# yuecideng/Misc3D

Hardware: AMD Instinct MI355X
Metric: RANSAC hypotheses/sec, 1M-pt cloud (inlier-score GB/s: roofline.algorithmic_reuse) (higher is better)
Workload: dtype f64 decisions (fp32 screen + fp64 recount)

## Files before the change

include/misc3d_amd_bench.h:

```cpp
#ifndef MISC3D_AMD_BENCH_H
#define MISC3D_AMD_BENCH_H

#include "misc3d_amd.h"

#ifdef __cplusplus
extern "C" {
#endif

int m3d_bench_time_score(m3d_cloud *cloud, int kind, double threshold, const uint32_t *samples,
                         size_t n_hypotheses, int reps, int mode, double *ms_avg,
                         uint64_t *listed_pairs);


int m3d_bench_fp64_issue_rate(int device, double ms_target, double *tera_lane_ops_per_s, double *ms_measured);

int m3d_bench_cloud_setup_ms(const m3d_cloud *cloud, double out[5]);

int m3d_bench_plane_upper_bounds(m3d_cloud *cloud, double threshold, const uint32_t *samples, size_t n_hypotheses,
                                 uint32_t *ub_out);
int m3d_bench_plane_ref_upper_bounds(m3d_cloud *cloud, double threshold, const uint32_t *samples, size_t n_hypotheses,
                                     size_t ref_index, uint32_t *ub_out);
int m3d_bench_upper_bounds(m3d_cloud *cloud, int kind, double threshold, const uint32_t *samples, size_t n_hypotheses,
                           uint32_t *ub_out);
int m3d_bench_last_segment_ms(double out[6]);

int m3d_bench_reg_checkers(const double *ps, const double *pd, const double *T, double edge_threshold,
                           double distance_threshold);

int m3d_bench_kabsch_sums(const double *src, const double *dst, size_t n, int device, double out[18]);

int m3d_bench_icp_sums(const double *src, size_t n_src, const double *dst, size_t n_dst, double max_correspondence_distance,
                       const double *T, int device, double out[29], int64_t *corr);

int m3d_bench_fps_force_path(int path);

int m3d_bench_knn_force_path(int path);

int m3d_bench_knn_tile_merge(const double *data, size_t n, int dim, const double *queries, size_t m, int kk, int pages,
                             int splits, uint32_t rows_per_split, int device, uint32_t *idx_out, uint64_t *d2_bits_out);

int m3d_bench_voxel_force_path(int path);

int m3d_bench_proximity_cutoffs(double dist, double angle_deg, double out[5]);

int m3d_bench_radius_grid_geom(const double lo[3], const double hi[3], double edge, int K0, int *K, double *h, uint64_t dims[3]);
int m3d_bench_reg_grid_k0(int k_cfg, uint64_t n_dst);

int m3d_bench_fpfh_pair_bins(const double *pairs, size_t m, int32_t *bins, double *features);

int m3d_bench_fpfh_stages(const double *xyz, const double *normals, size_t n, int search, double radius, int max_nn, int device,
                          uint32_t *list_idx, double *list_d2, uint32_t *cnt, uint8_t *spfh_count, double *spfh_incr,
                          uint32_t *tie_points, uint64_t *n_ties, double *feature_out, m3d_fpfh_stats *stats);

unsigned m3d_bench_match_last_path(void);

int m3d_bench_ppf_force(int device_memory_path, int max_groups);

int m3d_bench_ppf_cluster_force(int splits);

int m3d_bench_scratch_fill(int pattern);
int m3d_bench_scratch_fill_stats(uint64_t out[2]);
int m3d_bench_scratch_probe(int device, size_t bytes, unsigned char first_last[128]);

#ifdef __cplusplus
}
#endif
#endif
```

misc3d_amd/csrc/m3d_bench_hooks.cpp:

```cpp
#include "m3d_driver_internal.hpp"

#pragma clang fp contract(off)

using namespace m3d;

extern "C" {

int m3d_bench_last_segment_ms(double out[6]) {
    if (!out) return fail(M3D_ERR_INVALID_ARG, "null argument");
    for (int k = 0; k < 6; ++k) out[k] = g_seg_ms[k];
    return M3D_OK;
}

int m3d_bench_radius_grid_geom(const double lo[3], const double hi[3], double edge, int K0, int* K, double* h, uint64_t dims[3]) {
    if (!lo || !hi || !K || !h || !dims || !(edge > 0.0) || K0 < 1 || K0 > 16)
        return fail(M3D_ERR_INVALID_ARG, "invalid argument");
    const RadiusGridGeom g = radius_grid_geom(lo, hi, edge, K0);
    *K = g.K;
    *h = g.h;
    for (int k = 0; k < 3; ++k) dims[k] = g.dims[k];
    return M3D_OK;
}

int m3d_bench_reg_grid_k0(int k_cfg, uint64_t n_dst) { return reg_grid_k0(k_cfg, n_dst); }

int m3d_bench_cloud_setup_ms(const m3d_cloud* c, double out[5]) {
    if (!c || !out) return fail(M3D_ERR_INVALID_ARG, "null argument");
    for (int k = 0; k < 5; ++k) out[k] = c->setup_ms[k];
    return M3D_OK;
}

int m3d_bench_fp64_issue_rate(int device, double ms_target, double* tops, double* ms_measured) {
    if (!tops) return fail(M3D_ERR_INVALID_ARG, "invalid argument");
    LaneLock lane(device);
    DeviceCtx* ctx = lane.ctx;
    if (!ctx) return M3D_ERR_DEVICE;
    HIPCHK(hipSetDevice(ctx->device));
    RESERVE(ctx->small, 256);
    const int blocks = 256 * 8;
    auto run = [&](int iters, float* ms) -> int {
        HIPCHK(hipEventRecord(ctx->ev0, ctx->stream));
        launch_fp64_issue_probe(ctx->small.as<double>(), blocks, iters, ctx->stream);
        HIPCHK(hipEventRecord(ctx->ev1, ctx->stream));
        HIPCHK(hipGetLastError());
        HIPCHK(hipStreamSynchronize(ctx->stream));
        HIPCHK(hipEventElapsedTime(ms, ctx->ev0, ctx->ev1));
        return M3D_OK;
    };
    float ms = 0;
    int rc = run(256, &ms);
    if (rc != M3D_OK) return rc;
    rc = run(2048, &ms);
    if (rc != M3D_OK) return rc;
    const double per_iter = (double)ms / 2048.0;
    const int iters = (int)std::min(4.0e6, std::max(1024.0, (ms_target > 0 ? ms_target : 2.0) / std::max(per_iter, 1e-9)));
    rc = run(iters, &ms);
    if (rc != M3D_OK) return rc;
    const double ops = (double)blocks * 256.0 * 16.0 * (double)iters;
    *tops = ops / ((double)ms * 1e-3) / 1e12;
    if (ms_measured) *ms_measured = ms;
    return M3D_OK;
}

}
```

misc3d_amd/csrc/m3d_mask_expand.hpp:

```cpp
#pragma once

#include <cstddef>
#include <cstdint>
#include <thread>
#include <vector>

#if defined(__x86_64__)
#include <immintrin.h>
#endif

namespace m3d {

constexpr uint32_t kMaskTileWords = 32;

inline uint64_t mask_tile_prefix(const uint32_t* counts, uint32_t nb, uint64_t* prefix) {
    uint64_t s = 0;
    for (uint32_t t = 0; t < nb; ++t) {
        prefix[t] = s;
        s += counts[t];
    }
    prefix[nb] = s;
    return s;
}

inline void mask_split(const uint64_t* prefix, uint32_t nb, uint32_t parts, uint32_t* bounds) {
    const uint64_t total = prefix[nb];
    bounds[0] = 0;
    uint32_t t = 0;
    for (uint32_t k = 1; k < parts; ++k) {
        const uint64_t want = total * k / parts;
        while (t < nb && prefix[t] < want) ++t;
        bounds[k] = t;
    }
    bounds[parts] = nb;
}

namespace mask_detail {

inline uint64_t word_at(const uint64_t* mask, uint64_t w, uint64_t n) {
    const uint64_t m = mask[w];
    const uint64_t first = w * 64;
    return n - first >= 64 ? m : (m & ((1ull << (n - first)) - 1ull));
}

inline bool expand_scalar(const uint64_t* mask, uint64_t n, const uint64_t* prefix, uint32_t t0, uint32_t t1, uint64_t* dst) {
    const uint64_t n_words = (n + 63) / 64;
    for (uint32_t t = t0; t < t1; ++t) {
        uint64_t pos = prefix[t];
        const uint64_t end = prefix[t + 1];
        const uint64_t w0 = (uint64_t)t * kMaskTileWords, w1 = w0 + kMaskTileWords < n_words ? w0 + kMaskTileWords : n_words;
        for (uint64_t w = w0; w < w1; ++w) {
            uint64_t m = word_at(mask, w, n);
            if (!m) continue;
            if (pos + (uint64_t)__builtin_popcountll(m) > end) return false;
            const uint64_t b = w * 64;
            do {
                dst[pos++] = b + (uint64_t)__builtin_ctzll(m);
                m &= m - 1;
            } while (m);
        }
        if (pos != end) return false;
    }
    return true;
}

#if defined(__x86_64__)
__attribute__((target("avx512f,popcnt"))) inline bool expand_avx512(const uint64_t* mask, uint64_t n, const uint64_t* prefix,
                                                                uint32_t t0, uint32_t t1, uint64_t* dst) {
    const uint64_t n_words = (n + 63) / 64;
    const __m512i lane = _mm512_set_epi64(7, 6, 5, 4, 3, 2, 1, 0);
    const __m512i eight = _mm512_set1_epi64(8);
    for (uint32_t t = t0; t < t1; ++t) {
        uint64_t pos = prefix[t];
        const uint64_t end = prefix[t + 1];
        const uint64_t w0 = (uint64_t)t * kMaskTileWords, w1 = w0 + kMaskTileWords < n_words ? w0 + kMaskTileWords : n_words;
        for (uint64_t w = w0; w < w1; ++w) {
            const uint64_t m = word_at(mask, w, n);
            if (!m) continue;
            const uint64_t pc = (uint64_t)_mm_popcnt_u64(m);
            if (pos + pc > end) return false;
            __m512i v = _mm512_add_epi64(_mm512_set1_epi64((long long)(w * 64)), lane);
            uint64_t* d = dst + pos;
            if (m == ~0ull) {
                for (int k = 0; k < 8; ++k) {
                    _mm512_storeu_si512(d + 8 * k, v);
                    v = _mm512_add_epi64(v, eight);
                }
            } else {
                for (int k = 0; k < 8; ++k) {
                    const __mmask8 s = (__mmask8)(m >> (8 * k));
                    if (s) {
                        const __m512i c = _mm512_maskz_compress_epi64(s, v);
                        const unsigned c_n = (unsigned)_mm_popcnt_u32(s);
                        _mm512_mask_storeu_epi64(d, (__mmask8)((1u << c_n) - 1u), c);
                        d += c_n;
                    }
                    v = _mm512_add_epi64(v, eight);
                }
            }
            pos += pc;
        }
        if (pos != end) return false;
    }
    return true;
}
#endif

}

inline bool mask_have_avx512() {
#if defined(__x86_64__)
    static const bool have = __builtin_cpu_supports("avx512f") && __builtin_cpu_supports("popcnt");
    return have;
#else
    return false;
#endif
}

inline bool mask_expand_range(const uint64_t* mask, uint64_t n, const uint64_t* prefix, uint32_t t0, uint32_t t1, uint64_t* dst,
                              int path = -1) {
#if defined(__x86_64__)
    if (path != 0 && mask_have_avx512()) return mask_detail::expand_avx512(mask, n, prefix, t0, t1, dst);
#endif
    return mask_detail::expand_scalar(mask, n, prefix, t0, t1, dst);
}

inline bool mask_expand_threads(const uint64_t* mask, uint64_t n, const uint32_t* counts, uint64_t* dst, uint32_t writers,
                                int path = -1) {
    const uint32_t nb = (uint32_t)((n + 64ull * kMaskTileWords - 1) / (64ull * kMaskTileWords));
    if (writers < 1) writers = 1;
    std::vector<uint64_t> prefix(nb + 1);
    mask_tile_prefix(counts, nb, prefix.data());
    std::vector<uint32_t> bounds(writers + 1);
    mask_split(prefix.data(), nb, writers, bounds.data());
    std::vector<char> ok(writers, 1);
    std::vector<std::thread> th;
    for (uint32_t k = 1; k < writers; ++k)
        th.emplace_back([&, k] { ok[k] = mask_expand_range(mask, n, prefix.data(), bounds[k], bounds[k + 1], dst, path); });
    ok[0] = mask_expand_range(mask, n, prefix.data(), bounds[0], bounds[1], dst, path);
    for (auto& t : th) t.join();
    for (char c : ok)
        if (!c) return false;
    return true;
}

}
```

misc3d_amd/csrc/m3d_refine.cpp:

```cpp
#include "m3d_driver_internal.hpp"
#include "m3d_generalfit_fp.hpp"
#include "m3d_mask_expand.hpp"

#include <condition_variable>
#include <mutex>
#include <sched.h>

#pragma clang fp contract(off)

namespace m3d {

namespace {
class MaskPool {
public:
    static MaskPool& get() {
        static MaskPool* p = new MaskPool();
        return *p;
    }
    static uint32_t writer_cap() {
        const int lm = config().list_mask;
        uint32_t cap = lm >= 2 ? (uint32_t)lm : 8u;
        cpu_set_t set;
        CPU_ZERO(&set);
        if (sched_getaffinity(0, sizeof(set), &set) == 0) cap = std::min<uint32_t>(cap, (uint32_t)std::max(CPU_COUNT(&set), 1));
        return std::max<uint32_t>(cap, 1u);
    }
    void arm() {
        const uint32_t helpers = writer_cap() - 1;
        spin_us_.store(std::max(config().wait_spin_us, 0), std::memory_order_relaxed);
        if (helpers == 0) return;
        std::lock_guard<std::mutex> lk(mu_);
        try {
            while (threads_ < helpers) {
                std::thread(&MaskPool::helper, this, threads_).detach();
                ++threads_;
            }
        } catch (...) {
        }
        want_ = std::min(helpers, threads_);
        arm_seq_.fetch_add(1, std::memory_order_release);
        if (parked_) cv_.notify_all();
    }
    bool expand(const uint64_t* mask, uint64_t n, const uint32_t* counts, uint64_t* dst) {
        const uint32_t nb = (uint32_t)((n + 64ull * kMaskTileWords - 1) / (64ull * kMaskTileWords));
        if (nb == 0) return true;
        bool expected = false;
        if (!busy_.compare_exchange_strong(expected, true, std::memory_order_acquire)) {
            std::vector<uint64_t> prefix(nb + 1);
            mask_tile_prefix(counts, nb, prefix.data());
            return mask_expand_range(mask, n, prefix.data(), 0, nb, dst);
        }
        prefix_.resize(nb + 1);
        mask_tile_prefix(counts, nb, prefix_.data());
        const uint32_t ranges = std::min<uint32_t>(nb, 4u * writer_cap());
        bounds_.resize(ranges + 1);
        mask_split(prefix_.data(), nb, ranges, bounds_.data());
        mask_ = mask;
        n_ = n;
        dst_ = dst;
        failed_.store(false, std::memory_order_relaxed);
        done_.store(0, std::memory_order_relaxed);
        job_.store((uint64_t)ranges << 32, std::memory_order_release);
        work();
        while (done_.load(std::memory_order_acquire) != ranges) {
#if defined(__x86_64__) || defined(__i386__)
            __builtin_ia32_pause();
#endif
        }
        const bool ok = !failed_.load(std::memory_order_relaxed);
        busy_.store(false, std::memory_order_release);
        return ok;
    }

private:
    bool work() {
        bool any = false;
        for (;;) {
            const uint64_t v = job_.load(std::memory_order_relaxed);
            if ((v & 0xFFFFFFFFull) >= (v >> 32)) return any;
            const uint64_t c = job_.fetch_add(1, std::memory_order_acq_rel);
            const uint32_t k = (uint32_t)c, ranges = (uint32_t)(c >> 32);
            if (k >= ranges) return any;
            if (!mask_expand_range(mask_, n_, prefix_.data(), bounds_[k], bounds_[k + 1], dst_))
                failed_.store(true, std::memory_order_relaxed);
            done_.fetch_add(1, std::memory_order_release);
            any = true;
        }
    }
    void helper(uint32_t id) {
        uint64_t seen = 0;
        for (;;) {
            {
                std::unique_lock<std::mutex> lk(mu_);
                ++parked_;
                cv_.wait(lk, [&] { return arm_seq_.load(std::memory_order_relaxed) != seen && id < want_; });
                --parked_;
                seen = arm_seq_.load(std::memory_order_relaxed);
            }
            auto t0 = std::chrono::steady_clock::now();
            for (uint32_t spins = 1;; ++spins) {
                if (work()) t0 = std::chrono::steady_clock::now();
                const uint64_t a = arm_seq_.load(std::memory_order_relaxed);
                if (a != seen) {
                    seen = a;
                    t0 = std::chrono::steady_clock::now();
                }
                if ((spins & 0xFFu) == 0 &&
                    std::chrono::duration_cast<std::chrono::microseconds>(std::chrono::steady_clock::now() - t0).count() >=
                        spin_us_.load(std::memory_order_relaxed))
                    break;
#if defined(__x86_64__) || defined(__i386__)
                __builtin_ia32_pause();
#endif
            }
        }
    }
    std::mutex mu_;
    std::condition_variable cv_;
    uint32_t threads_ = 0, want_ = 0, parked_ = 0;
    std::atomic<uint64_t> arm_seq_{0};
    std::atomic<int> spin_us_{0};
    std::atomic<bool> busy_{false};
    std::atomic<uint64_t> job_{0};
    std::atomic<uint32_t> done_{0};
    std::atomic<bool> failed_{false};
    const uint64_t* mask_ = nullptr;
    uint64_t n_ = 0;
    uint64_t* dst_ = nullptr;
    std::vector<uint64_t> prefix_;
    std::vector<uint32_t> bounds_;
};
}


int compact_scratch(DeviceCtx* ctx, uint32_t nb, uint32_t** slots) {
    RESERVE(ctx->block_counts, sizeof(uint32_t) * ((size_t)nb + 1));
    *slots = ctx->block_counts.as<uint32_t>();
    return M3D_OK;
}

int exact_error(DeviceCtx* ctx, const CloudView& v, int kind, double thr,
                       const double* model_dev, uint64_t* count, double* error) {
    const uint32_t nb = (v.n + kCompactTile - 1) / kCompactTile;
    RESERVE(ctx->dist, sizeof(double) * (size_t)std::max<uint32_t>(v.n, 1));
    uint32_t* scratch;
    if (const int rc = compact_scratch(ctx, nb, &scratch); rc != M3D_OK) return rc;
    RESERVE(ctx->total, sizeof(uint32_t) * 4);
    RESERVE(ctx->sums, sizeof(double) * 32);
    RESERVE(ctx->h_small, 256);
    launch_compact(kind, v, model_dev, thr, 1, nullptr, nullptr, ctx->dist.as<double>(), nullptr,
                   nullptr, nullptr, nullptr, 0, scratch,
                   ctx->total.as<uint32_t>(), ctx->stream);
    launch_serial_sum(ctx->dist.as<double>(), ctx->total.as<uint32_t>(), ctx->sums.as<double>() + 16,
                      ctx->stream);
    uint8_t* h = ctx->h_small.as<uint8_t>();
    HIPCHK(hipMemcpyAsync(h, ctx->total.p, sizeof(uint32_t), hipMemcpyDeviceToHost, ctx->stream));
    HIPCHK(hipMemcpyAsync(h + 8, ctx->sums.as<double>() + 16, sizeof(double), hipMemcpyDeviceToHost,
                          ctx->stream));
    HIPCHK(hipGetLastError());
    HIPCHK(hipStreamSynchronize(ctx->stream));
    uint32_t c32;
    std::memcpy(&c32, h, 4);
    std::memcpy(error, h + 8, 8);
    *count = c32;
    return M3D_OK;
}

int approx_error_pair(DeviceCtx* ctx, const CloudView& v, int kind, double thr, const double* model_a,
                             const double* model_b, uint64_t* count_a, double* error_a, uint64_t* count_b, double* error_b) {
    const bool fresh = ctx->tie_scratch.cap == 0;
    RESERVE(ctx->tie_scratch, sizeof(double) * (kErrorSumScratchDoubles + 2));
    RESERVE(ctx->h_tie, 64);
    uint32_t* ticket = reinterpret_cast<uint32_t*>(ctx->tie_scratch.as<double>() + kErrorSumScratchDoubles);
    if (fresh) HIPCHK(hipMemsetAsync(ticket, 0, sizeof(uint32_t), ctx->stream));
    double* h = ctx->h_tie.as<double>();
    launch_error_sum(kind, v, model_a, model_b, thr, ctx->tie_scratch.as<double>(), ticket, h, ctx->stream);
    HIPCHK(hipGetLastError());
    HIPCHK(hipStreamSynchronize(ctx->stream));
    *count_a = (uint64_t)h[0];
    *error_a = h[1];
    if (model_b) {
        *count_b = (uint64_t)h[2];
        *error_b = h[3];
    }
    return M3D_OK;
}
int approx_error(DeviceCtx* ctx, const CloudView& v, int kind, double thr,
                        const double* model_dev, uint64_t* count, double* error) {
    return approx_error_pair(ctx, v, kind, thr, model_dev, nullptr, count, error, nullptr, nullptr);
}


static uint64_t* idx_dev(DeviceCtx* ctx, const FitCaller* fc) { return fc && fc->idx_dev ? fc->idx_dev : ctx->idx.as<uint64_t>(); }

int issue_refine_compaction(DeviceCtx* ctx, const CloudView& flag_view, const uint32_t* orig_dev, int kind, double thr,
                            const double* model_dev, const double* lazy_in, void* total_host, const FitCaller* fc,
                            Compaction* out, bool fused, uint64_t* idx_host, const PartitionOut* part, bool allow_mask) {
    const uint32_t n = flag_view.n;
    const uint32_t nb = (n + kCompactTile - 1) / kCompactTile;
    RESERVE(ctx->idx, sizeof(uint64_t) * (size_t)std::max<uint32_t>(n, 1));
    uint32_t* scratch;
    if (const int rc = compact_scratch(ctx, nb, &scratch); rc != M3D_OK) return rc;
    RESERVE(ctx->total, sizeof(uint32_t) * 4);
    fused = fused && kind != M3D_CYLINDER;
    if (fused) {
        RESERVE(ctx->moment_partial, sizeof(double) * 16 * (size_t)std::max<uint32_t>(nb, 1));
        RESERVE(ctx->h_moments, sizeof(double) * 2 * kFusedMomentDoubles);
    }
    const bool early = config().mask_early != 0;
    const bool mask = allow_mask && fused && idx_host && nb && !orig_dev && !part && !(fc && (fc->idx_dev || fc->defer_refine)) &&
                      config().list_mask != 0;
    if (mask) {
        RESERVE(ctx->h_mask, sizeof(uint64_t) * kMaskTileWords * (size_t)nb);
        RESERVE(ctx->h_tile_counts, sizeof(uint32_t) * (size_t)nb);
        if (!ctx->h_sync.p) {
            RESERVE(ctx->h_sync, 64);
            std::memset(ctx->h_sync.p, 0, 64);
        }
        if (++ctx->mask_seq == 0) ++ctx->mask_seq;
        MaskPool::get().arm();
    }
    launch_compact(kind, flag_view, model_dev, thr, 0, orig_dev,
                   idx_dev(ctx, fc), nullptr,
                   nullptr, nullptr, nullptr, nullptr, 0, scratch,
                   ctx->total.as<uint32_t>(), ctx->stream, const_cast<double*>(lazy_in),
                   fused ? ctx->moment_partial.as<double>() : nullptr, fused ? h_moments_at(ctx, refine_slot(fc)) : nullptr,
                   idx_host, static_cast<uint32_t*>(total_host) , part,
                   mask ? ctx->h_mask.as<uint64_t>() : nullptr, mask ? ctx->h_tile_counts.as<uint32_t>() : nullptr,
                   mask ? ctx->h_sync.as<uint32_t>() + 1 : nullptr, ctx->mask_seq,
                   mask && early ? ctx->h_sync.as<uint32_t>() + 2 : nullptr);
    *out = Compaction{};
    out->total = total_host;
    out->fused = fused;
    out->idx_host = idx_host;
    out->mask = mask;
    out->mask_early = mask && early;
    return M3D_OK;
}

static bool expand_compaction_mask(DeviceCtx* ctx, uint32_t n, uint32_t expected, uint64_t* dst) {
    const uint32_t nb = (n + kCompactTile - 1) / kCompactTile;
    const uint32_t* counts = ctx->h_tile_counts.as<const uint32_t>();
    uint64_t total = 0;
    for (uint32_t t = 0; t < nb; ++t) total += counts[t];
    if (total != expected) return false;
    return MaskPool::get().expand(ctx->h_mask.as<const uint64_t>(), n, counts, dst);
}

static int fit_from_moments(int kind, const double* mean, const double* moments, uint32_t ni, double* params_host) {
    double out[4];
    if (!(kind == M3D_PLANE ? plane_from_moments(mean, moments, out) : sphere_from_moments(mean, moments, (double)ni, out))) return 0;
    std::memcpy(params_host, out, sizeof(out));
    return 1;
}

static int refine_in_order(DeviceCtx* ctx, const CloudView& flag_view, const CloudView& gather_view, const uint32_t* orig_dev,
                           int kind, double thr, const double* model_dev, double* params_host, size_t* inliers, size_t* n_inliers,
                           int* general_fit_ok, Compaction cp, const FitCaller* fc, bool hook_due, const double* lazy_in) {
    if (!cp.total) {
        const PartitionOut* part = fc && fc->partition_hook && orig_dev ? (*fc->partition_hook)(-1) : nullptr;
        const int rc = issue_refine_compaction(ctx, flag_view, orig_dev, kind, thr, model_dev, lazy_in, ctx->h_small.p, fc, &cp,
                                               false, nullptr, part, false);
        if (rc != M3D_OK) return rc;
    }
    const bool idx_on_host = inliers && cp.idx_host == reinterpret_cast<uint64_t*>(inliers);
    HIPCHK(hipGetLastError());
    if (hook_due && fc && fc->before_refine_wait) {
        const int hr = (*fc->before_refine_wait)(-1);
        if (hr != M3D_OK) return hr;
    }
    HIPCHK(hipStreamSynchronize(ctx->stream));
    if (lazy_in) std::memcpy(params_host, lazy_in, sizeof(double) * kModelStride);
    uint32_t ni;
    std::memcpy(&ni, cp.total, 4);
    *n_inliers = ni;
    *general_fit_ok = 1;
    const bool need_fit = kind != M3D_CYLINDER;
    const uint32_t min_pts = kind == M3D_PLANE ? 3 : 4;
    if (need_fit) {
        if (ni < min_pts) {
            *general_fit_ok = 0;
        } else {
            launch_general_fit_sums(gather_view, idx_dev(ctx, fc), ni, ctx->sum_partial.as<double>(),
                                    ctx->h_sums.as<double>(), ctx->stream);
        }
    }
    if (inliers && ni && !idx_on_host)
        HIPCHK(hipMemcpyAsync(inliers, (void*)idx_dev(ctx, fc), sizeof(uint64_t) * (size_t)ni,
                              hipMemcpyDeviceToHost, ctx->stream));
    HIPCHK(hipGetLastError());
    HIPCHK(hipStreamSynchronize(ctx->stream));
    if (need_fit && *general_fit_ok) {
        double sums[14];
        general_fit_sums_finish(ctx->h_sums.as<double>(), sums);
        const double mean[3] = {sums[0] / (double)ni, sums[1] / (double)ni, sums[2] / (double)ni};
        *general_fit_ok = fit_from_moments(kind, mean, sums + 4, ni, params_host);
    }
    return M3D_OK;
}

int refine(DeviceCtx* ctx, const CloudView& flag_view, const CloudView& gather_view, const uint32_t* orig_dev, int kind, double thr,
           const double* model_dev, double* params_host, size_t* inliers, size_t* n_inliers, int* general_fit_ok, int64_t expected_ni,
           const Compaction& queued, const FitCaller* fc, bool hook_due, const double* lazy_in, bool fused) {
    const uint32_t n = flag_view.n;
    fused = fused && lazy_in != nullptr;
    RESERVE(ctx->sums, sizeof(double) * 32);
    RESERVE(ctx->sum_partial, sizeof(double) * kSumPartialDoubles);
    RESERVE(ctx->h_sums, sizeof(double) * kGeneralFitHostDoubles);
    RESERVE(ctx->h_small, 256);
    Compaction cp = queued;
    if (!cp.total) {
        uint64_t* idx_host = inliers && fused && !(fc && fc->idx_dev) &&
                                     is_library_pinned(inliers, sizeof(uint64_t) * (size_t)std::max<uint32_t>(n, 1))
                                 ? reinterpret_cast<uint64_t*>(inliers) : nullptr;
        const PartitionOut* part = fc && fc->partition_hook && orig_dev ? (*fc->partition_hook)(expected_ni) : nullptr;
        const int rc = issue_refine_compaction(ctx, flag_view, orig_dev, kind, thr, model_dev, lazy_in, ctx->h_small.p, fc, &cp,
                                               fused, idx_host, part, expected_ni >= 0);
        if (rc != M3D_OK) return rc;
    }
    const bool have_moments = fused && cp.fused;
    const bool idx_on_host = inliers && cp.idx_host == reinterpret_cast<uint64_t*>(inliers);
    const bool expected = expected_ni >= 0 && (uint64_t)expected_ni <= n;
    if (cp.mask && !(idx_on_host && expected))
        return refine_in_order(ctx, flag_view, gather_view, orig_dev, kind, thr, model_dev, params_host, inliers, n_inliers,
                               general_fit_ok, Compaction{}, fc, hook_due, lazy_in);
    if (!expected)
        return refine_in_order(ctx, flag_view, gather_view, orig_dev, kind, thr, model_dev, params_host, inliers, n_inliers,
                               general_fit_ok, cp, fc, hook_due, lazy_in);
    const uint32_t ni_e = (uint32_t)expected_ni;
    const bool need_fit_e = kind != M3D_CYLINDER && ni_e >= (kind == M3D_PLANE ? 3u : 4u);
    if (!cp.ev_recorded) HIPCHK(hipEventRecord(ctx->ev_compact, ctx->stream));
    const bool early_copy = !idx_on_host && inliers && ni_e && is_library_pinned(inliers, sizeof(uint64_t) * (size_t)ni_e);
    if (early_copy) {
        HIPCHK(hipStreamWaitEvent(copy_stream_of(ctx), ctx->ev_compact, 0));
        HIPCHK(hipMemcpyAsync(inliers, (void*)idx_dev(ctx, fc),
                              sizeof(uint64_t) * (size_t)ni_e, hipMemcpyDeviceToHost, copy_stream_of(ctx)));
    }
    if (need_fit_e && !have_moments) {
        launch_general_fit_sums(gather_view, idx_dev(ctx, fc), ni_e, ctx->sum_partial.as<double>(),
                                ctx->h_sums.as<double>(), ctx->stream);
    }
    const bool hooked = hook_due && fc && fc->before_refine_wait;
    if (hooked) {
        const int hr = (*fc->before_refine_wait)(expected_ni);
        if (hr != M3D_OK) return hr;
    }
    if (inliers && ni_e && !early_copy && !idx_on_host) {
        HIPCHK(hipStreamWaitEvent(copy_stream_of(ctx), ctx->ev_compact, 0));
        HIPCHK(hipMemcpyAsync(inliers, (void*)idx_dev(ctx, fc),
                              sizeof(uint64_t) * (size_t)ni_e, hipMemcpyDeviceToHost, copy_stream_of(ctx)));
    }
    HIPCHK(hipGetLastError());
    bool expanded = false, expand_ok = true;
    if (hooked && (have_moments || !need_fit_e)) {
        HIPCHK(hipEventSynchronize(ctx->ev_compact));
    } else if (cp.mask && !hooked) {
        if (cp.mask_early && ni_e) {
            const int erc = word_wait_spin(ctx, ctx->h_sync.as<uint32_t>() + 2, ctx->mask_seq);
            if (erc != M3D_OK) return erc;
            expand_ok = expand_compaction_mask(ctx, n, ni_e, reinterpret_cast<uint64_t*>(inliers));
            expanded = true;
        }
        const int wrc = word_wait_spin(ctx, ctx->h_sync.as<uint32_t>() + 1, ctx->mask_seq);
        if (wrc != M3D_OK) return wrc;
    } else {
        const int wrc = stream_wait_spin(ctx);
        if (wrc != M3D_OK) return wrc;
    }
    const bool list_on_copy_stream = inliers && ni_e && !idx_on_host;
    if (list_on_copy_stream && !(fc && fc->defer_copy_sync && fc->idx_dev)) HIPCHK(hipStreamSynchronize(copy_stream_of(ctx)));
    if (lazy_in) std::memcpy(params_host, lazy_in, sizeof(double) * kModelStride);
    uint32_t ni_chk;
    std::memcpy(&ni_chk, cp.total, 4);
    if (ni_chk != ni_e ||
        (cp.mask && ni_e && !(expanded ? expand_ok : expand_compaction_mask(ctx, n, ni_e, reinterpret_cast<uint64_t*>(inliers)))))
        return refine_in_order(ctx, flag_view, gather_view, orig_dev, kind, thr, model_dev, params_host, inliers, n_inliers,
                               general_fit_ok, Compaction{}, fc, false, nullptr);
    *n_inliers = ni_e;
    *general_fit_ok = 1;
    if (kind != M3D_CYLINDER && !need_fit_e) {
        *general_fit_ok = 0;
    } else if (kind != M3D_CYLINDER) {
        double sums[14];
        double mean[3];
        if (have_moments) {
            const double* rec = lazy_in;
            const double c0[3] = {rec[4], rec[5], rec[6]};
            moments_about_mean(h_moments_at(ctx, refine_slot(fc)), c0, (double)ni_e, mean, sums + 4);
        } else {
            general_fit_sums_finish(ctx->h_sums.as<double>(), sums);
            for (int k = 0; k < 3; ++k) mean[k] = sums[k] / (double)ni_e;
        }
        *general_fit_ok = fit_from_moments(kind, mean, sums + 4, ni_e, params_host);
    }
    return M3D_OK;
}

}

using namespace m3d;

extern "C" {

int m3d_cloud_exact_error(m3d_cloud* c, int kind, double threshold, const double* model,
                          uint64_t* count, double* error) {
    if (!c || kind < 0 || kind > 2 || !model || !count || !error)
        return fail(M3D_ERR_INVALID_ARG, "invalid argument");
    DeviceCtx* ctx = c->ctx;
    CtxLock lock(ctx);
    HIPCHK(hipSetDevice(ctx->device));
    RESERVE(ctx->small, 256);
    double tmp[kModelStride] = {0, 0, 0, 0, 0, 0, 0, 0};
    std::memcpy(tmp, model, sizeof(double) * num_params(kind));
    HIPCHK(hipMemcpyAsync(ctx->small.p, tmp, sizeof(tmp), hipMemcpyHostToDevice, ctx->stream));
    HIPCHK(hipStreamSynchronize(ctx->stream));
    return exact_error(ctx, c->view(), kind, threshold, ctx->small.as<double>(), count, error);
}

int m3d_cloud_refine_expect(m3d_cloud* c, int kind, double threshold, double* params, int64_t expected_inliers,
                            size_t* inliers, size_t* n_inliers) {
    if (!c || kind < 0 || kind > 2 || !params || !n_inliers)
        return fail(M3D_ERR_INVALID_ARG, "invalid argument");
    DeviceCtx* ctx = c->ctx;
    CtxLock lock(ctx);
    HIPCHK(hipSetDevice(ctx->device));
    RESERVE(ctx->small, 256);
    RESERVE(ctx->h_small, 256);
    double tmp[kModelStride] = {0, 0, 0, 0, 0, 0, 0, 0};
    std::memcpy(tmp, params, sizeof(double) * num_params(kind));
    std::memcpy(ctx->h_small.as<uint8_t>() + 192, tmp, sizeof(tmp));
    HIPCHK(hipMemcpyAsync(ctx->small.p, ctx->h_small.as<uint8_t>() + 192, sizeof(tmp), hipMemcpyHostToDevice, ctx->stream));
    int gf = 1;
    const CloudView v = c->view();
    const int rc = refine(ctx, v, c->base_view(), c->orig(), kind, threshold, ctx->small.as<double>(), tmp, inliers,
                          n_inliers, &gf, expected_inliers, Compaction{}, nullptr);
    if (rc != M3D_OK) return rc;
    std::memcpy(params, tmp, sizeof(double) * num_params(kind));
    return gf ? M3D_OK : M3D_FALSE;
}
int m3d_cloud_refine(m3d_cloud* c, int kind, double threshold, double* params, size_t* inliers,
                     size_t* n_inliers) {
    return m3d_cloud_refine_expect(c, kind, threshold, params, -1, inliers, n_inliers);
}


}
```

Before: 59.10 million.

## Split host mask expansion by output cache lines and pin helpers to shared-LLC cores

```diff
diff --git a/include/misc3d_amd_bench.h b/include/misc3d_amd_bench.h
--- a/include/misc3d_amd_bench.h
+++ b/include/misc3d_amd_bench.h
@@ -15,6 +15,8 @@
 int m3d_bench_fp64_issue_rate(int device, double ms_target, double *tera_lane_ops_per_s, double *ms_measured);
 
 int m3d_bench_cloud_setup_ms(const m3d_cloud *cloud, double out[5]);
+
+int m3d_bench_host_block(const void *p, size_t bytes);
 
 int m3d_bench_plane_upper_bounds(m3d_cloud *cloud, double threshold, const uint32_t *samples, size_t n_hypotheses,
                                  uint32_t *ub_out);
diff --git a/misc3d_amd/csrc/m3d_bench_hooks.cpp b/misc3d_amd/csrc/m3d_bench_hooks.cpp
--- a/misc3d_amd/csrc/m3d_bench_hooks.cpp
+++ b/misc3d_amd/csrc/m3d_bench_hooks.cpp
@@ -5,6 +5,8 @@
 using namespace m3d;
 
 extern "C" {
+
+int m3d_bench_host_block(const void* p, size_t bytes) { return p && is_library_pinned(p, bytes) ? 1 : 0; }
 
 int m3d_bench_last_segment_ms(double out[6]) {
     if (!out) return fail(M3D_ERR_INVALID_ARG, "null argument");
diff --git a/misc3d_amd/csrc/m3d_mask_expand.hpp b/misc3d_amd/csrc/m3d_mask_expand.hpp
--- a/misc3d_amd/csrc/m3d_mask_expand.hpp
+++ b/misc3d_amd/csrc/m3d_mask_expand.hpp
@@ -37,7 +37,7 @@
 
 namespace mask_detail {
 
-inline uint64_t word_at(const uint64_t* mask, uint64_t w, uint64_t n) {
+__attribute__((always_inline)) inline uint64_t word_at(const uint64_t* mask, uint64_t w, uint64_t n) {
     const uint64_t m = mask[w];
     const uint64_t first = w * 64;
     return n - first >= 64 ? m : (m & ((1ull << (n - first)) - 1ull));
@@ -106,6 +106,135 @@
 }
 #endif
 
+
+__attribute__((always_inline)) inline bool tile_agrees(const uint64_t* mask, uint64_t n, const uint64_t* prefix, uint32_t t, uint64_t* w0, uint64_t* w1) {
+    const uint64_t n_words = (n + 63) / 64;
+    *w0 = (uint64_t)t * kMaskTileWords;
+    *w1 = *w0 + kMaskTileWords < n_words ? *w0 + kMaskTileWords : n_words;
+    uint64_t c = 0;
+    for (uint64_t w = *w0; w < *w1; ++w) c += (uint64_t)__builtin_popcountll(word_at(mask, w, n));
+    return c == prefix[t + 1] - prefix[t];
+}
+inline uint32_t tile_of(const uint64_t* prefix, uint32_t nb, uint64_t p) {
+    uint32_t lo = 0, hi = nb;
+    while (lo < hi) {
+        const uint32_t mid = lo + (hi - lo) / 2;
+        if (prefix[mid + 1] > p) hi = mid; else lo = mid + 1;
+    }
+    return lo;
+}
+__attribute__((always_inline)) inline uint64_t cut_word(uint64_t m, uint64_t skip, uint64_t room) {
+    for (; skip && m; --skip) m &= m - 1;
+    while (m && (uint64_t)__builtin_popcountll(m) > room) m &= ~(1ull << (63 - __builtin_clzll(m)));
+    return m;
+}
+
+struct SpanTiles {
+    const uint64_t* mask;
+    uint64_t n;
+    const uint64_t* prefix;
+    uint32_t nb;
+    uint64_t p0, p1;
+    uint32_t t;
+    bool ok = true;
+    SpanTiles(const uint64_t* mask_, uint64_t n_, const uint64_t* prefix_, uint32_t nb_, uint64_t p0_, uint64_t p1_)
+        : mask(mask_), n(n_), prefix(prefix_), nb(nb_), p0(p0_), p1(p1_), t(nb_) {
+        if (p0 >= p1) return;
+        if (p1 > prefix[nb]) {
+            ok = false;
+            return;
+        }
+        t = tile_of(prefix, nb, p0);
+        if (prefix[t] == p0)
+            while (t > 0 && prefix[t - 1] == p0) --t;
+    }
+    __attribute__((always_inline)) inline bool next(uint64_t* w0, uint64_t* w1, uint64_t* first, bool* whole) {
+        for (;;) {
+            if (t >= nb) return false;
+            const bool empty = prefix[t + 1] == prefix[t];
+            if (prefix[t] >= p1 && !(empty && p1 == prefix[nb])) return false;
+            if (!tile_agrees(mask, n, prefix, t, w0, w1)) {
+                ok = false;
+                return false;
+            }
+            ++t;
+            if (empty) continue;
+            *first = prefix[t - 1];
+            *whole = prefix[t - 1] >= p0 && prefix[t] <= p1;
+            return true;
+        }
+    }
+    __attribute__((always_inline)) inline uint64_t cut(uint64_t m, uint64_t* pos, uint64_t* after) const {
+        const uint64_t first = *pos, pc = (uint64_t)__builtin_popcountll(m);
+        *after = first + pc;
+        if (first + pc <= p0 || first >= p1) return 0;
+        const uint64_t skip = first < p0 ? p0 - first : 0;
+        *pos = first + skip;
+        return (skip || first + pc > p1) ? cut_word(m, skip, p1 - (first + skip)) : m;
+    }
+};
+
+inline bool span_scalar(const uint64_t* mask, uint64_t n, const uint64_t* prefix, uint32_t nb, uint64_t p0, uint64_t p1, uint64_t* dst) {
+    SpanTiles tiles(mask, n, prefix, nb, p0, p1);
+    uint64_t w0, w1, pos;
+    bool whole;
+    while (tiles.next(&w0, &w1, &pos, &whole))
+        for (uint64_t w = w0; w < w1; ++w) {
+            uint64_t m = word_at(mask, w, n);
+            if (!m) continue;
+            uint64_t after = 0;
+            if (!whole) m = tiles.cut(m, &pos, &after);
+            for (const uint64_t b = w * 64; m; m &= m - 1) dst[pos++] = b + (uint64_t)__builtin_ctzll(m);
+            if (!whole) pos = after;
+        }
+    return tiles.ok;
+}
+
+#if defined(__x86_64__)
+__attribute__((target("avx512f,popcnt"))) inline bool span_avx512_masked(const uint64_t* mask, uint64_t n, const uint64_t* prefix,
+                                                                         uint32_t nb, uint64_t p0, uint64_t p1, uint64_t* dst) {
+    const __m512i lane = _mm512_set_epi64(7, 6, 5, 4, 3, 2, 1, 0);
+    const __m512i eight = _mm512_set1_epi64(8);
+    SpanTiles tiles(mask, n, prefix, nb, p0, p1);
+    uint64_t w0, w1, pos;
+    bool whole;
+    while (tiles.next(&w0, &w1, &pos, &whole))
+        for (uint64_t w = w0; w < w1; ++w) {
+            uint64_t m = word_at(mask, w, n);
+            if (!m) continue;
+            uint64_t after = 0;
+            if (!whole) {
+                m = tiles.cut(m, &pos, &after);
+                if (!m) {
+                    pos = after;
+                    continue;
+                }
+            }
+            __m512i v = _mm512_add_epi64(_mm512_set1_epi64((long long)(w * 64)), lane);
+            uint64_t* d = dst + pos;
+            if (m == ~0ull) {
+                for (int k = 0; k < 8; ++k) {
+                    _mm512_storeu_si512(d, v);
+                    d += 8;
+                    v = _mm512_add_epi64(v, eight);
+                }
+            } else {
+                for (int k = 0; k < 8; ++k) {
+                    const __mmask8 s = (__mmask8)(m >> (8 * k));
+                    if (s) {
+                        const unsigned c_n = (unsigned)_mm_popcnt_u32(s);
+                        _mm512_mask_storeu_epi64(d, (__mmask8)((1u << c_n) - 1u), _mm512_maskz_compress_epi64(s, v));
+                        d += c_n;
+                    }
+                    v = _mm512_add_epi64(v, eight);
+                }
+            }
+            pos = whole ? (uint64_t)(d - dst) : after;
+        }
+    return tiles.ok;
+}
+#endif
+
 }
 
 inline bool mask_have_avx512() {
@@ -123,6 +252,26 @@
     if (path != 0 && mask_have_avx512()) return mask_detail::expand_avx512(mask, n, prefix, t0, t1, dst);
 #endif
     return mask_detail::expand_scalar(mask, n, prefix, t0, t1, dst);
+}
+
+inline void mask_split_lines(uint64_t total, uint32_t parts, const uint64_t* dst, uint64_t* cuts) {
+    const uint64_t a = ((uintptr_t)dst >> 3) & 7u;
+    cuts[0] = 0;
+    for (uint32_t k = 1; k < parts; ++k) {
+        uint64_t c = (total * k / parts + a + 4) & ~7ull;
+        c = c > a ? c - a : 0;
+        if (c > total) c = total;
+        cuts[k] = c < cuts[k - 1] ? cuts[k - 1] : c;
+    }
+    cuts[parts] = total;
+}
+
+inline bool mask_expand_span(const uint64_t* mask, uint64_t n, const uint64_t* prefix, uint32_t nb, uint64_t p0, uint64_t p1,
+                             uint64_t* dst, int path = -1) {
+#if defined(__x86_64__)
+    if (path != 0 && mask_have_avx512()) return mask_detail::span_avx512_masked(mask, n, prefix, nb, p0, p1, dst);
+#endif
+    return mask_detail::span_scalar(mask, n, prefix, nb, p0, p1, dst);
 }
 
 inline bool mask_expand_threads(const uint64_t* mask, uint64_t n, const uint32_t* counts, uint64_t* dst, uint32_t writers,
@@ -144,4 +293,23 @@
     return true;
 }
 
-}
+inline bool mask_expand_spans_threads(const uint64_t* mask, uint64_t n, const uint32_t* counts, uint64_t* dst, uint32_t writers,
+                                      int path = -1) {
+    const uint32_t nb = (uint32_t)((n + 64ull * kMaskTileWords - 1) / (64ull * kMaskTileWords));
+    if (writers < 1) writers = 1;
+    std::vector<uint64_t> prefix(nb + 1);
+    const uint64_t total = mask_tile_prefix(counts, nb, prefix.data());
+    std::vector<uint64_t> cuts(writers + 1);
+    mask_split_lines(total, writers, dst, cuts.data());
+    std::vector<char> ok(writers, 1);
+    std::vector<std::thread> th;
+    for (uint32_t k = 1; k < writers; ++k)
+        th.emplace_back([&, k] { ok[k] = mask_expand_span(mask, n, prefix.data(), nb, cuts[k], cuts[k + 1], dst, path); });
+    ok[0] = mask_expand_span(mask, n, prefix.data(), nb, cuts[0], cuts[1], dst, path);
+    for (auto& t : th) t.join();
+    for (char c : ok)
+        if (!c) return false;
+    return true;
+}
+
+}
diff --git a/misc3d_amd/csrc/m3d_mask_pool.hpp b/misc3d_amd/csrc/m3d_mask_pool.hpp
--- /dev/null
+++ b/misc3d_amd/csrc/m3d_mask_pool.hpp
@@ -0,0 +1,247 @@
+#pragma once
+
+#include "m3d_mask_expand.hpp"
+
+#include <algorithm>
+#include <atomic>
+#include <chrono>
+#include <condition_variable>
+#include <cstdio>
+#include <cstdlib>
+#include <map>
+#include <string>
+#include <mutex>
+#include <sched.h>
+#include <thread>
+#include <vector>
+
+namespace m3d {
+
+namespace mask_detail {
+inline std::vector<int> read_cpu_list(const char* path) {
+    std::vector<int> out;
+    FILE* f = std::fopen(path, "r");
+    if (!f) return out;
+    char buf[4096];
+    const size_t got = std::fread(buf, 1, sizeof(buf) - 1, f);
+    std::fclose(f);
+    buf[got] = 0;
+    const char* p = buf;
+    while (*p >= '0' && *p <= '9') {
+        char* e;
+        const long a = std::strtol(p, &e, 10);
+        long b = a;
+        if (*e == '-') b = std::strtol(e + 1, &e, 10);
+        if (a < 0 || b < a || b - a > 4096) return std::vector<int>();
+        for (long c = a; c <= b; ++c) out.push_back((int)c);
+        p = *e == ',' ? e + 1 : e;
+    }
+    return out;
+}
+}
+
+class MaskPool {
+public:
+    std::string sysfs_cpu = "/sys/devices/system/cpu";
+
+    static MaskPool& get() {
+        static MaskPool* p = new MaskPool();
+        return *p;
+    }
+    static uint32_t writer_cap(int list_mask) {
+        uint32_t cap = list_mask >= 2 ? (uint32_t)list_mask : 8u;
+        cpu_set_t set;
+        CPU_ZERO(&set);
+        if (sched_getaffinity(0, sizeof(set), &set) == 0) cap = std::min<uint32_t>(cap, (uint32_t)std::max(CPU_COUNT(&set), 1));
+        return std::max<uint32_t>(cap, 1u);
+    }
+    void arm(uint32_t writers, int spin_us) {
+        const uint32_t helpers = writers ? writers - 1 : 0;
+        spin_us_.store(std::max(spin_us, 0), std::memory_order_relaxed);
+        if (helpers == 0) return;
+        std::lock_guard<std::mutex> lk(mu_);
+        place(helpers);
+        try {
+            while (threads_ < helpers) {
+                std::thread(&MaskPool::helper, this, threads_).detach();
+                ++threads_;
+            }
+        } catch (...) {
+        }
+        want_ = std::min(helpers, threads_);
+        arm_seq_.fetch_add(1, std::memory_order_release);
+        if (parked_) cv_.notify_all();
+    }
+    bool expand(const uint64_t* mask, uint64_t n, const uint32_t* counts, uint64_t* dst, uint32_t writers) {
+        const uint32_t nb = (uint32_t)((n + 64ull * kMaskTileWords - 1) / (64ull * kMaskTileWords));
+        if (nb == 0) return true;
+        bool expected = false;
+        if (!busy_.compare_exchange_strong(expected, true, std::memory_order_acquire)) {
+            std::vector<uint64_t> prefix(nb + 1);
+            const uint64_t total = mask_tile_prefix(counts, nb, prefix.data());
+            return mask_expand_span(mask, n, prefix.data(), nb, 0, total, dst);
+        }
+        prefix_.resize(nb + 1);
+        const uint64_t total = mask_tile_prefix(counts, nb, prefix_.data());
+        const uint32_t spans = std::min<uint32_t>(nb, 4u * std::max<uint32_t>(writers, 1u));
+        cuts_.resize(spans + 1);
+        mask_split_lines(total, spans, dst, cuts_.data());
+        mask_ = mask;
+        n_ = n;
+        nb_ = nb;
+        dst_ = dst;
+        failed_.store(false, std::memory_order_relaxed);
+        done_.store(0, std::memory_order_relaxed);
+        job_.store((uint64_t)spans << 32, std::memory_order_release);
+        work();
+        while (done_.load(std::memory_order_acquire) != spans) {
+#if defined(__x86_64__) || defined(__i386__)
+            __builtin_ia32_pause();
+#endif
+        }
+        const bool ok = !failed_.load(std::memory_order_relaxed);
+        busy_.store(false, std::memory_order_release);
+        return ok;
+    }
+
+private:
+    bool work() {
+        bool any = false;
+        for (;;) {
+            const uint64_t v = job_.load(std::memory_order_relaxed);
+            if ((v & 0xFFFFFFFFull) >= (v >> 32)) return any;
+            const uint64_t c = job_.fetch_add(1, std::memory_order_acq_rel);
+            const uint32_t k = (uint32_t)c, spans = (uint32_t)(c >> 32);
+            if (k >= spans) return any;
+            if (!mask_expand_span(mask_, n_, prefix_.data(), nb_, cuts_[k], cuts_[k + 1], dst_))
+                failed_.store(true, std::memory_order_relaxed);
+            done_.fetch_add(1, std::memory_order_release);
+            any = true;
+        }
+    }
+    void place(uint32_t helpers) {
+        const int cpu = sched_getcpu();
+        if (cpu < 0) return;
+        if ((size_t)cpu < llc_of_.size() && llc_of_[cpu] == placed_llc_ && placed_for_ >= helpers &&
+            std::find(given_.begin(), given_.end(), cpu) == given_.end())
+            return;
+        if ((size_t)cpu >= llc_of_.size()) llc_of_.resize((size_t)cpu + 1, -2);
+        if (llc_of_[cpu] == -2) {
+            char path[512];
+            std::snprintf(path, sizeof(path), "%s/cpu%d/cache/index3/shared_cpu_list", sysfs_cpu.c_str(), cpu);
+            std::vector<int> group = mask_detail::read_cpu_list(path);
+            const int id = group.empty() ? -1 : group[0];
+            for (int c : group) {
+                if ((size_t)c >= llc_of_.size()) llc_of_.resize((size_t)c + 1, -2);
+                llc_of_[c] = id;
+            }
+            llc_of_[cpu] = id;
+            if (id >= 0 && !groups_.count(id)) {
+                cpu_set_t mine;
+                CPU_ZERO(&mine);
+                if (sched_getaffinity(0, sizeof(mine), &mine) != 0) group.clear();
+                std::vector<std::pair<int, int>> keyed;
+                for (int c : group) {
+                    if (c >= CPU_SETSIZE || !CPU_ISSET(c, &mine)) continue;
+                    std::snprintf(path, sizeof(path), "%s/cpu%d/topology/thread_siblings_list", sysfs_cpu.c_str(), c);
+                    const std::vector<int> sib = mask_detail::read_cpu_list(path);
+                    const int rank = (int)(std::find(sib.begin(), sib.end(), c) - sib.begin());
+                    keyed.emplace_back(sib.empty() ? 0 : rank, c);
+                }
+                std::sort(keyed.begin(), keyed.end());
+                std::vector<int>& g = groups_[id];
+                for (const auto& kc : keyed) g.push_back(kc.second);
+            }
+        }
+        const int id = llc_of_[cpu];
+        placed_llc_ = id;
+        placed_for_ = helpers;
+        if (id < 0) return;
+        const std::vector<int>& g = groups_[id];
+        std::vector<int> order;
+        char path[512];
+        std::snprintf(path, sizeof(path), "%s/cpu%d/topology/thread_siblings_list", sysfs_cpu.c_str(), cpu);
+        const std::vector<int> own = mask_detail::read_cpu_list(path);
+        for (int c : g)
+            if (c != cpu && std::find(own.begin(), own.end(), c) == own.end()) order.push_back(c);
+        if (bind_.size() < helpers) bind_.resize(helpers);
+        given_.clear();
+        cpu_set_t anywhere;
+        CPU_ZERO(&anywhere);
+        if (sched_getaffinity(0, sizeof(anywhere), &anywhere) != 0) return;
+        for (uint32_t h = 0; h < helpers; ++h) {
+            cpu_set_t& s = bind_[h];
+            CPU_ZERO(&s);
+            if (h >= order.size()) {
+                s = anywhere;
+            } else {
+                CPU_SET(order[h], &s);
+                given_.push_back(order[h]);
+            }
+        }
+        bind_seq_.fetch_add(1, std::memory_order_release);
+    }
+    void helper(uint32_t id) {
+        uint64_t seen = 0, bound = 0;
+        for (;;) {
+            {
+                std::unique_lock<std::mutex> lk(mu_);
+                ++parked_;
+                cv_.wait(lk, [&] { return arm_seq_.load(std::memory_order_relaxed) != seen && id < want_; });
+                --parked_;
+                seen = arm_seq_.load(std::memory_order_relaxed);
+                rebind(id, &bound);
+            }
+            auto t0 = std::chrono::steady_clock::now();
+            for (uint32_t spins = 1;; ++spins) {
+                if (work()) t0 = std::chrono::steady_clock::now();
+                const uint64_t a = arm_seq_.load(std::memory_order_relaxed);
+                if (a != seen) {
+                    seen = a;
+                    t0 = std::chrono::steady_clock::now();
+                    if (bind_seq_.load(std::memory_order_acquire) != bound) {
+                        std::lock_guard<std::mutex> lk(mu_);
+                        rebind(id, &bound);
+                    }
+                }
+                if ((spins & 0xFFu) == 0 &&
+                    std::chrono::duration_cast<std::chrono::microseconds>(std::chrono::steady_clock::now() - t0).count() >=
+                        spin_us_.load(std::memory_order_relaxed))
+                    break;
+#if defined(__x86_64__) || defined(__i386__)
+                __builtin_ia32_pause();
+#endif
+            }
+        }
+    }
+    void rebind(uint32_t id, uint64_t* bound) {
+        const uint64_t b = bind_seq_.load(std::memory_order_acquire);
+        if (b == *bound) return;
+        *bound = b;
+        if (id < bind_.size() && CPU_COUNT(&bind_[id]) > 0) (void)sched_setaffinity(0, sizeof(cpu_set_t), &bind_[id]);
+    }
+    std::mutex mu_;
+    std::condition_variable cv_;
+    uint32_t threads_ = 0, want_ = 0, parked_ = 0;
+    std::vector<int> llc_of_;
+    std::map<int, std::vector<int>> groups_;
+    std::vector<cpu_set_t> bind_;
+    std::vector<int> given_;
+    int placed_llc_ = -3;
+    uint32_t placed_for_ = 0;
+    std::atomic<uint64_t> bind_seq_{0};
+    std::atomic<uint64_t> arm_seq_{0};
+    std::atomic<int> spin_us_{0};
+    std::atomic<bool> busy_{false};
+    std::atomic<uint64_t> job_{0};
+    std::atomic<uint32_t> done_{0};
+    std::atomic<bool> failed_{false};
+    const uint64_t* mask_ = nullptr;
+    uint64_t n_ = 0;
+    uint32_t nb_ = 0;
+    uint64_t* dst_ = nullptr;
+    std::vector<uint64_t> prefix_;
+    std::vector<uint64_t> cuts_;
+};
+
+}
diff --git a/misc3d_amd/csrc/m3d_refine.cpp b/misc3d_amd/csrc/m3d_refine.cpp
--- a/misc3d_amd/csrc/m3d_refine.cpp
+++ b/misc3d_amd/csrc/m3d_refine.cpp
@@ -1,137 +1,12 @@
 #include "m3d_driver_internal.hpp"
 #include "m3d_generalfit_fp.hpp"
-#include "m3d_mask_expand.hpp"
-
-#include <condition_variable>
-#include <mutex>
-#include <sched.h>
+#include "m3d_mask_pool.hpp"
 
 #pragma clang fp contract(off)
 
 namespace m3d {
 
-namespace {
-class MaskPool {
-public:
-    static MaskPool& get() {
-        static MaskPool* p = new MaskPool();
-        return *p;
-    }
-    static uint32_t writer_cap() {
-        const int lm = config().list_mask;
-        uint32_t cap = lm >= 2 ? (uint32_t)lm : 8u;
-        cpu_set_t set;
-        CPU_ZERO(&set);
-        if (sched_getaffinity(0, sizeof(set), &set) == 0) cap = std::min<uint32_t>(cap, (uint32_t)std::max(CPU_COUNT(&set), 1));
-        return std::max<uint32_t>(cap, 1u);
-    }
-    void arm() {
-        const uint32_t helpers = writer_cap() - 1;
-        spin_us_.store(std::max(config().wait_spin_us, 0), std::memory_order_relaxed);
-        if (helpers == 0) return;
-        std::lock_guard<std::mutex> lk(mu_);
-        try {
-            while (threads_ < helpers) {
-                std::thread(&MaskPool::helper, this, threads_).detach();
-                ++threads_;
-            }
-        } catch (...) {
-        }
-        want_ = std::min(helpers, threads_);
-        arm_seq_.fetch_add(1, std::memory_order_release);
-        if (parked_) cv_.notify_all();
-    }
-    bool expand(const uint64_t* mask, uint64_t n, const uint32_t* counts, uint64_t* dst) {
-        const uint32_t nb = (uint32_t)((n + 64ull * kMaskTileWords - 1) / (64ull * kMaskTileWords));
-        if (nb == 0) return true;
-        bool expected = false;
-        if (!busy_.compare_exchange_strong(expected, true, std::memory_order_acquire)) {
-            std::vector<uint64_t> prefix(nb + 1);
-            mask_tile_prefix(counts, nb, prefix.data());
-            return mask_expand_range(mask, n, prefix.data(), 0, nb, dst);
-        }
-        prefix_.resize(nb + 1);
-        mask_tile_prefix(counts, nb, prefix_.data());
-        const uint32_t ranges = std::min<uint32_t>(nb, 4u * writer_cap());
-        bounds_.resize(ranges + 1);
-        mask_split(prefix_.data(), nb, ranges, bounds_.data());
-        mask_ = mask;
-        n_ = n;
-        dst_ = dst;
-        failed_.store(false, std::memory_order_relaxed);
-        done_.store(0, std::memory_order_relaxed);
-        job_.store((uint64_t)ranges << 32, std::memory_order_release);
-        work();
-        while (done_.load(std::memory_order_acquire) != ranges) {
-#if defined(__x86_64__) || defined(__i386__)
-            __builtin_ia32_pause();
-#endif
-        }
-        const bool ok = !failed_.load(std::memory_order_relaxed);
-        busy_.store(false, std::memory_order_release);
-        return ok;
-    }
-
-private:
-    bool work() {
-        bool any = false;
-        for (;;) {
-            const uint64_t v = job_.load(std::memory_order_relaxed);
-            if ((v & 0xFFFFFFFFull) >= (v >> 32)) return any;
-            const uint64_t c = job_.fetch_add(1, std::memory_order_acq_rel);
-            const uint32_t k = (uint32_t)c, ranges = (uint32_t)(c >> 32);
-            if (k >= ranges) return any;
-            if (!mask_expand_range(mask_, n_, prefix_.data(), bounds_[k], bounds_[k + 1], dst_))
-                failed_.store(true, std::memory_order_relaxed);
-            done_.fetch_add(1, std::memory_order_release);
-            any = true;
-        }
-    }
-    void helper(uint32_t id) {
-        uint64_t seen = 0;
-        for (;;) {
-            {
-                std::unique_lock<std::mutex> lk(mu_);
-                ++parked_;
-                cv_.wait(lk, [&] { return arm_seq_.load(std::memory_order_relaxed) != seen && id < want_; });
-                --parked_;
-                seen = arm_seq_.load(std::memory_order_relaxed);
-            }
-            auto t0 = std::chrono::steady_clock::now();
-            for (uint32_t spins = 1;; ++spins) {
-                if (work()) t0 = std::chrono::steady_clock::now();
-                const uint64_t a = arm_seq_.load(std::memory_order_relaxed);
-                if (a != seen) {
-                    seen = a;
-                    t0 = std::chrono::steady_clock::now();
-                }
-                if ((spins & 0xFFu) == 0 &&
-                    std::chrono::duration_cast<std::chrono::microseconds>(std::chrono::steady_clock::now() - t0).count() >=
-                        spin_us_.load(std::memory_order_relaxed))
-                    break;
-#if defined(__x86_64__) || defined(__i386__)
-                __builtin_ia32_pause();
-#endif
-            }
-        }
-    }
-    std::mutex mu_;
-    std::condition_variable cv_;
-    uint32_t threads_ = 0, want_ = 0, parked_ = 0;
-    std::atomic<uint64_t> arm_seq_{0};
-    std::atomic<int> spin_us_{0};
-    std::atomic<bool> busy_{false};
-    std::atomic<uint64_t> job_{0};
-    std::atomic<uint32_t> done_{0};
-    std::atomic<bool> failed_{false};
-    const uint64_t* mask_ = nullptr;
-    uint64_t n_ = 0;
-    uint64_t* dst_ = nullptr;
-    std::vector<uint64_t> prefix_;
-    std::vector<uint32_t> bounds_;
-};
-}
-
+static uint32_t mask_writers() { return MaskPool::writer_cap(config().list_mask); }
 
 int compact_scratch(DeviceCtx* ctx, uint32_t nb, uint32_t** slots) {
     RESERVE(ctx->block_counts, sizeof(uint32_t) * ((size_t)nb + 1));
@@ -218,7 +93,7 @@
             std::memset(ctx->h_sync.p, 0, 64);
         }
         if (++ctx->mask_seq == 0) ++ctx->mask_seq;
-        MaskPool::get().arm();
+        MaskPool::get().arm(mask_writers(), config().wait_spin_us);
     }
     launch_compact(kind, flag_view, model_dev, thr, 0, orig_dev,
                    idx_dev(ctx, fc), nullptr,
@@ -244,7 +119,7 @@
     uint64_t total = 0;
     for (uint32_t t = 0; t < nb; ++t) total += counts[t];
     if (total != expected) return false;
-    return MaskPool::get().expand(ctx->h_mask.as<const uint64_t>(), n, counts, dst);
+    return MaskPool::get().expand(ctx->h_mask.as<const uint64_t>(), n, counts, dst, mask_writers());
 }
 
 static int fit_from_moments(int kind, const double* mean, const double* moments, uint32_t ni, double* params_host) {
```

Measured after the change: 65.22 million, median of 6. 10.4% higher.
